# gitvicky/CP-PRE

Hardware: AMD Instinct MI355X
Metric: residual-cells/s (PRE eval+calibrate) (higher is better)
Workload: dtype f32

## Files before the change

cp_pre_amd/csrc/star_march.h:

```cpp
#pragma once
#include "common.h"
#include "host_checks.h"
#include <atomic>
#include <type_traits>

namespace {

constexpr int MAXF = 6;

struct Geom {
    const float *f[MAXF];
    long long sB[MAXF], sT[MAXF], sX[MAXF];
    float *out;
    long long oB, oT, oX;
    int B, T, X, Y;
    int Yc;
    int tSeg, nTSeg, nXT, nYT;
    int flags;
    int flat;
    int tfree;
    int obuf;
};

struct Star { float c, tm, tp, xm, xp, ym, yp; };

struct Nbr { float4 c, tm, tp, xm, xp, ym, yp; };

__device__ __forceinline__ float4 f4(float s) { return make_float4(s, s, s, s); }
__device__ __forceinline__ float4 fabs4(const float4 &a) { return make_float4(fabsf(a.x), fabsf(a.y), fabsf(a.z), fabsf(a.w)); }

enum Kind { K_T3, K_X3, K_Y3, K_XY5, K_TX5, K_STAR7, K_TY5 };

template <int KIND>
__device__ __forceinline__ float4 apply(const Star &w, const Nbr &n)
{
    if (KIND == K_T3) return w.tm * n.tm + w.c * n.c + w.tp * n.tp;
    if (KIND == K_X3) return w.xm * n.xm + w.c * n.c + w.xp * n.xp;
    if (KIND == K_Y3) return w.ym * n.ym + w.c * n.c + w.yp * n.yp;
    if (KIND == K_XY5) return w.xm * n.xm + w.ym * n.ym + w.c * n.c + w.yp * n.yp + w.xp * n.xp;
    if (KIND == K_TX5) return w.tm * n.tm + w.xm * n.xm + w.c * n.c + w.xp * n.xp + w.tp * n.tp;
    if (KIND == K_TY5) return w.tm * n.tm + w.ym * n.ym + w.c * n.c + w.yp * n.yp + w.tp * n.tp;
    const float4 tm = w.tm != 0.f ? w.tm * n.tm : f4(0.f), tp = w.tp != 0.f ? w.tp * n.tp : f4(0.f);
    return tm + w.xm * n.xm + w.ym * n.ym + w.c * n.c + w.yp * n.yp + w.xp * n.xp + tp;
}

template <int MODE> struct OpKinds {
    static constexpr int DT = MODE == 2 ? K_STAR7 : (MODE >= 3 ? K_Y3 : K_T3);
    static constexpr int DX = MODE == 2 ? K_STAR7 : (MODE >= 3 ? K_T3 : K_X3);
    static constexpr int DY = MODE == 2 ? K_STAR7 : (MODE == 0 ? K_T3 : MODE == 1 ? K_Y3 : MODE == 3 ? K_Y3 : K_X3);
    static constexpr int LAP = MODE == 2 ? K_STAR7 : (MODE >= 3 ? K_TX5 : K_XY5);
};

enum { O_DT = 1, O_DX = 2, O_DY = 4, O_LAP = 8 };
constexpr bool kind_has_x(int k) { return k == K_X3 || k == K_XY5 || k == K_TX5 || k == K_STAR7; }
template <int MODE> constexpr bool ops_have_x(int ops)
{
    using K = OpKinds<MODE>;
    return ((ops & O_DT) && kind_has_x(K::DT)) || ((ops & O_DX) && kind_has_x(K::DX)) || ((ops & O_DY) && kind_has_x(K::DY)) ||
           ((ops & O_LAP) && kind_has_x(K::LAP));
}
template <int MODE> constexpr unsigned xmask_of(int o0, int o1 = 0, int o2 = 0, int o3 = 0, int o4 = 0, int o5 = 0)
{
    return (ops_have_x<MODE>(o0) ? 1u : 0u) | (ops_have_x<MODE>(o1) ? 2u : 0u) | (ops_have_x<MODE>(o2) ? 4u : 0u) |
           (ops_have_x<MODE>(o3) ? 8u : 0u) | (ops_have_x<MODE>(o4) ? 16u : 0u) | (ops_have_x<MODE>(o5) ? 32u : 0u);
}

struct Linear1 {
    static constexpr int F = 1;
    struct Params { Star s; };
    static __device__ __forceinline__ float4 eval(const Nbr (&n)[1], const Params &p) { return apply<K_STAR7>(p.s, n[0]); }
};

struct Linear2 {
    static constexpr int F = 2;
    struct Params { Star a, b; float ratio; };
    static __device__ __forceinline__ float4 eval(const Nbr (&n)[2], const Params &p)
    {
        return apply<K_STAR7>(p.a, n[0]) + p.ratio * apply<K_STAR7>(p.b, n[1]);
    }
};

struct NSParams { Star Dt, Dx, Dy, L; float dxdy, dtdy, dtdx, nudt; };
struct BurgersParams { Star Dt, Dx, Dxx; float dx, dt, nu, c3; };
struct MHDParams { Star Dt, Dx, Dy; float gamma, gm2; };

template <int MODE>
struct NSMomentum {
    static constexpr int F = 3;
    static constexpr int MIN_WAVES = MODE >= 3 ? 4 : 1;
    static constexpr bool HALO_LEAD = MODE == 0;
    static constexpr unsigned XMASK = xmask_of<MODE>(O_DT | O_DX | O_DY | O_LAP, O_DT | O_DX | O_DY | O_LAP, O_DX | O_DY);
    using Params = NSParams;
    static __device__ __forceinline__ float4 eval(const Nbr (&n)[3], const Params &p)
    {
        using K = OpKinds<MODE>;
        const Nbr &u = n[0], &v = n[1], &pr = n[2];
        float4 rx = apply<K::DT>(p.Dt, u) * p.dxdy;
        rx = rx + u.c * apply<K::DX>(p.Dx, u) * p.dtdy;
        rx = rx + v.c * apply<K::DY>(p.Dy, u) * p.dtdx;
        rx = rx - apply<K::LAP>(p.L, u) * p.nudt;
        rx = rx + apply<K::DX>(p.Dx, pr) * p.dtdy;
        float4 ry = apply<K::DT>(p.Dt, v) * p.dxdy;
        ry = ry + u.c * apply<K::DX>(p.Dx, v) * p.dtdx;
        ry = ry + v.c * apply<K::DY>(p.Dy, v) * p.dtdy;
        ry = ry - apply<K::LAP>(p.L, v) * p.nudt;
        ry = ry + apply<K::DY>(p.Dy, pr) * p.dtdx;
        return rx + ry;
    }
};

template <int MODE>
struct Burgers {
    static constexpr int F = 1;
    using Params = BurgersParams;
    static __device__ __forceinline__ float4 eval(const Nbr (&n)[1], const Params &p)
    {
        constexpr int KT = MODE == 0 ? K_X3 : MODE == 3 ? K_Y3 : K_STAR7, KX = MODE == 0 ? K_Y3 : MODE == 3 ? K_X3 : K_STAR7;
        const Nbr &u = n[0];
        float4 r = p.dx * apply<KT>(p.Dt, u);
        r = r + (p.dt * u.c) * apply<KX>(p.Dx, u);
        r = r - (p.nu * apply<KX>(p.Dxx, u)) * p.c3;
        return r;
    }
};

template <int MODE>
struct MHDContinuity {
    static constexpr int F = 3;
    static constexpr unsigned XMASK = xmask_of<MODE>(O_DT | O_DX | O_DY, O_DX, O_DY);
    using Params = MHDParams;
    static __device__ __forceinline__ float4 eval(const Nbr (&n)[3], const Params &p)
    {
        using K = OpKinds<MODE>;
        const Nbr &rho = n[0], &u = n[1], &v = n[2];
        float4 r = apply<K::DT>(p.Dt, rho) + u.c * apply<K::DX>(p.Dx, rho);
        r = r + rho.c * apply<K::DX>(p.Dx, u);
        r = r + v.c * apply<K::DY>(p.Dy, rho);
        r = r + rho.c * apply<K::DY>(p.Dy, v);
        return r;
    }
};

template <int MODE>
struct MHDMomentum {
    static constexpr int F = 6;
    static constexpr unsigned XMASK = xmask_of<MODE>(0, O_DT | O_DX | O_DY, O_DT | O_DX | O_DY, O_DX | O_DY, O_DX | O_DY, O_DX | O_DY);
    using Params = MHDParams;
    static __device__ __forceinline__ float4 eval(const Nbr (&n)[6], const Params &p)
    {
        using K = OpKinds<MODE>;
        const Nbr &rho = n[0], &u = n[1], &v = n[2], &pr = n[3], &bx = n[4], &by = n[5];
        const float4 irho = f4(1.0f) / rho.c, bxr = bx.c / rho.c, byr = by.c / rho.c;
        float4 rx = apply<K::DT>(p.Dt, u) + u.c * apply<K::DX>(p.Dx, u);
        rx = rx + irho * apply<K::DX>(p.Dx, pr);
        rx = rx - (2.0f * bxr) * apply<K::DX>(p.Dx, bx);
        rx = rx + v.c * apply<K::DY>(p.Dy, u);
        rx = rx - byr * apply<K::DY>(p.Dy, bx);
        rx = rx - bxr * apply<K::DY>(p.Dy, by);
        float4 ry = apply<K::DT>(p.Dt, v) + u.c * apply<K::DX>(p.Dx, v);
        ry = ry + irho * apply<K::DY>(p.Dy, pr);
        ry = ry - (2.0f * byr) * apply<K::DY>(p.Dy, by);
        ry = ry + v.c * apply<K::DY>(p.Dy, v);
        ry = ry - byr * apply<K::DX>(p.Dx, bx);
        ry = ry - bxr * apply<K::DX>(p.Dx, by);
        return rx + ry;
    }
};

template <int MODE>
struct MHDEnergy {
    static constexpr int F = 6;
    static constexpr unsigned XMASK = xmask_of<MODE>(O_DT, O_DX | O_DY, O_DX | O_DY, O_DX | O_DY, O_DX, O_DY);
    using Params = MHDParams;
    static __device__ __forceinline__ float4 eval(const Nbr (&n)[6], const Params &p)
    {
        using K = OpKinds<MODE>;
        const Nbr &rho = n[0], &u = n[1], &v = n[2], &pr = n[3], &bx = n[4], &by = n[5];
        const float4 bx2 = bx.c * bx.c, by2 = by.c * by.c;
        const float4 pgas = pr.c - 0.5f * (bx2 + by2);
        float4 r = apply<K::DT>(p.Dt, rho) + u.c * apply<K::DX>(p.Dx, pr);
        r = r + v.c * apply<K::DY>(p.Dy, pr);
        r = r + (p.gm2 * (u.c * bx.c + v.c * by.c)) * (apply<K::DX>(p.Dx, bx) + apply<K::DY>(p.Dy, by));
        r = r + (p.gamma * pgas + by2) * apply<K::DX>(p.Dx, u);
        r = r + (p.gamma * pgas + bx2) * apply<K::DY>(p.Dy, v);
        r = r - (bx.c * by.c) * (apply<K::DY>(p.Dy, u) + apply<K::DX>(p.Dx, v));
        return r;
    }
};

template <int MODE>
struct MHDInduction {
    static constexpr int F = 4;
    static constexpr unsigned XMASK = xmask_of<MODE>(O_DX | O_DY, O_DX | O_DY, O_DT | O_DX | O_DY, O_DT | O_DX | O_DY);
    using Params = MHDParams;
    static __device__ __forceinline__ float4 eval(const Nbr (&n)[4], const Params &p)
    {
        using K = OpKinds<MODE>;
        const Nbr &u = n[0], &v = n[1], &bx = n[2], &by = n[3];
        float4 rx = apply<K::DT>(p.Dt, bx) - by.c * apply<K::DY>(p.Dy, u);
        rx = rx + bx.c * apply<K::DY>(p.Dy, v);
        rx = rx - v.c * apply<K::DY>(p.Dy, bx);
        rx = rx + u.c * apply<K::DY>(p.Dy, by);
        float4 ry = apply<K::DT>(p.Dt, by) + by.c * apply<K::DX>(p.Dx, u);
        ry = ry - bx.c * apply<K::DX>(p.Dx, v);
        ry = ry - v.c * apply<K::DX>(p.Dx, bx);
        ry = ry + u.c * apply<K::DX>(p.Dx, by);
        return rx + ry;
    }
};

struct JorekParams { Star Dt, DR, DZ, DRR, DZZ; float a0, a1, a2, a3; };

template <int MODE>
struct JorekContinuity {
    static constexpr int F = 3;
    static constexpr unsigned XMASK = xmask_of<MODE>(O_DT | O_DX | O_DY, O_DX | O_DY, 0);
    using Params = JorekParams;
    static __device__ __forceinline__ float4 eval(const Nbr (&n)[3], const Params &p)
    {
        using K = OpKinds<MODE>;
        const Nbr &rho = n[0], &phi = n[1];
        const float4 R = n[2].c;
        const float4 dRrho = apply<K::DX>(p.DR, rho), dZphi = apply<K::DY>(p.DZ, phi);
        const float4 X = dRrho * dZphi - apply<K::DX>(p.DR, phi) * apply<K::DY>(p.DZ, rho);
        const float4 Y = (apply<K::DX>(p.DRR, rho) + (f4(1.0f) / R) * dRrho) + apply<K::DY>(p.DZZ, rho);
        float4 r = p.a0 * apply<K::DT>(p.Dt, rho);
        r = r - (p.a1 * R) * X;
        r = r - (p.a2 * rho.c) * dZphi;
        r = r - p.a3 * Y;
        return r;
    }
};

template <int MODE>
struct JorekTemperature {
    static constexpr int F = 4;
    static constexpr unsigned XMASK = xmask_of<MODE>(O_DT | O_DX | O_DY, O_DX | O_DY, O_DT | O_DX | O_DY, 0);
    using Params = JorekParams;
    static __device__ __forceinline__ float4 eval(const Nbr (&n)[4], const Params &p)
    {
        using K = OpKinds<MODE>;
        const Nbr &rho = n[0], &phi = n[1], &T = n[2];
        const float4 R = n[3].c;
        const float4 dZphi = apply<K::DY>(p.DZ, phi), dRphi = apply<K::DX>(p.DR, phi);
        const float4 dRT = apply<K::DX>(p.DR, T);
        const float4 XT = dRT * dZphi - dRphi * apply<K::DY>(p.DZ, T);
        const float4 Xr = apply<K::DX>(p.DR, rho) * dZphi - dRphi * apply<K::DY>(p.DZ, rho);
        const float4 YT = (apply<K::DX>(p.DRR, T) + (f4(1.0f) / R) * dRT) + apply<K::DY>(p.DZZ, T);
        float4 r = T.c * apply<K::DT>(p.Dt, rho) + rho.c * apply<K::DT>(p.Dt, T);
        r = r - (rho.c * R) * XT;
        r = r + (T.c * R) * Xr;
        r = r + ((p.a0 * rho.c) * T.c) * dZphi;
        r = r + p.a3 * YT;
        return r;
    }
};

struct __attribute__((aligned(4))) F4u { float x, y, z, w; };
__device__ __forceinline__ float4 ldg4(const float *p)
{
    const F4u v = *reinterpret_cast<const F4u *>(p);
    return make_float4(v.x, v.y, v.z, v.w);
}
__device__ __forceinline__ void stg4(float *p, const float4 &r) { *reinterpret_cast<F4u *>(p) = F4u{r.x, r.y, r.z, r.w}; }

#ifndef MARCH_ST_SC1
#define MARCH_ST_SC1 0
#endif
__device__ __forceinline__ void stb4_sc1(float *plane, unsigned int off, const float4 &r)
{
    typedef unsigned int u32x4 __attribute__((ext_vector_type(4)));
    const u32x4 v = {__float_as_uint(r.x), __float_as_uint(r.y), __float_as_uint(r.z), __float_as_uint(r.w)};
    __builtin_amdgcn_raw_buffer_store_b128(v, __builtin_amdgcn_make_buffer_rsrc(plane, 0, -1, 0x00020000), (int)off, 0, 16);
}

#ifndef MARCH_DPP
#define MARCH_DPP 0
#endif
__device__ __forceinline__ float lane_below(float x)
{
#if MARCH_DPP
    return __int_as_float(__builtin_amdgcn_update_dpp(0, __float_as_int(x), 0x138, 0xf, 0xf, false));
#else
    return __shfl_up(x, 1);
#endif
}
__device__ __forceinline__ float lane_above(float x)
{
#if MARCH_DPP
    return __int_as_float(__builtin_amdgcn_update_dpp(0, __float_as_int(x), 0x130, 0xf, 0xf, false));
#else
    return __shfl_down(x, 1);
#endif
}

__device__ __forceinline__ void lds_barrier()
{
    __builtin_amdgcn_fence(__ATOMIC_RELEASE, "workgroup", "local");
    __builtin_amdgcn_s_barrier();
    __builtin_amdgcn_fence(__ATOMIC_ACQUIRE, "workgroup", "local");
}

template <int F, bool BC, bool COOP> struct Halo {
    typename std::conditional<COOP, float, float4>::type row[F];
    float ye[F];
    float yr[BC ? F : 1];
};

struct NoBC {};

#ifndef MARCH6_NR
#define MARCH6_NR 8
#endif
#ifndef MARCH6_TYQ
#define MARCH6_TYQ 64
#endif
#ifndef MARCH6_MINW
#define MARCH6_MINW 1
#endif
#ifndef MARCH1_TSEG
#define MARCH1_TSEG 0
#endif
#ifndef MARCHN_TSEG
#define MARCHN_TSEG 0
#endif
#ifndef TFREE_TSEG
#define TFREE_TSEG 8
#endif
#ifndef MARCH1_ANYB
#define MARCH1_ANYB 0
#endif
#ifndef MARCH6_AHEAD
#define MARCH6_AHEAD 2
#endif
#ifndef MARCH_COOP_MAXF
#define MARCH_COOP_MAXF 4
#endif
#ifndef MARCH_HALO_AHEAD
#define MARCH_HALO_AHEAD 1
#endif
#ifndef MARCH_NS16
#define MARCH_NS16 0
#endif

template <class Fn, class = void> struct MinWaves { static constexpr int value = Fn::F >= 5 ? MARCH6_MINW : 1; };
template <class Fn> struct MinWaves<Fn, std::void_t<decltype(Fn::MIN_WAVES)>> { static constexpr int value = Fn::MIN_WAVES; };

template <class Fn, class = void> struct HaloLead { static constexpr bool value = MARCH_HALO_AHEAD == 2; };
template <class Fn> struct HaloLead<Fn, std::void_t<decltype(Fn::HALO_LEAD)>> {
    static constexpr bool value = MARCH_HALO_AHEAD == 2 || (MARCH_HALO_AHEAD == 1 && Fn::HALO_LEAD);
};

template <class Fn, class = void> struct XMask { static constexpr unsigned value = (1u << Fn::F) - 1u; };
template <class Fn> struct XMask<Fn, std::void_t<decltype(Fn::XMASK)>> { static constexpr unsigned value = Fn::XMASK & ((1u << Fn::F) - 1u); };
template <class Fn> struct Staged {
    static constexpr unsigned M = XMask<Fn>::value;
    static constexpr int count = __builtin_popcount(M);
    static constexpr int FX = count > 0 ? count : 1;
    static __device__ __forceinline__ constexpr bool has(int i) { return (M >> i) & 1u; }
    static __device__ __forceinline__ constexpr int slot(int i) { return __builtin_popcount(M & ((1u << i) - 1u)); }
};

template <class Fn, int NR, int TYQ, bool BC = false>
__global__ void __launch_bounds__(NR *TYQ, MinWaves<Fn>::value)
march_kernel(const Geom g, const typename Fn::Params prm, const typename std::conditional<BC, BCInfo, NoBC>::type bc)
{
    constexpr int F = Fn::F;
    using SX = Staged<Fn>;
    constexpr int AHEAD = (F >= 5 && MARCH6_AHEAD == 3) ? 3 : 2;
    constexpr bool HAL3 = HaloLead<Fn>::value && !BC && F <= MARCH_COOP_MAXF && AHEAD == 2;
    static_assert(NR >= 2, "tile needs at least two rows (top and bottom halo owners differ)");
    __shared__ float4 lds[2][SX::FX][NR + 2][TYQ];

    const int q = threadIdx.x, ty = threadIdx.y;
    unsigned L = xcd_remap(blockIdx.x, gridDim.x);
    const int yt = L % g.nYT; L /= g.nYT;
    const int xt = L % g.nXT; L /= g.nXT;
    const int ts = L % g.nTSeg;
    const int b = L / g.nTSeg;

    const int x = xt * NR + ty, y = (yt * TYQ + q) * 4;
    const bool inb = (x < g.X) && (y < g.Yc);
    int xl = x;
    float ghost = 0.f;
    bool ldown = inb;
    if constexpr (BC) {
        if (x == g.X && y < g.Yc) { xl = bc.xhi; ghost = bc.vxhi; ldown = bc.xhi >= 0; }
    } else {
        if ((g.flags & PRE_FLAG_HALO_X) && x == g.X && y < g.Yc) ldown = true;
    }
    int t0 = ts * g.tSeg;
    int t1 = min(t0 + g.tSeg, g.T);
    if (g.flags & PRE_FLAG_INTERIOR_T) {
        t0 = max(t0, 1);
        t1 = min(t1, g.T - 1);
    }

    static_assert(NR >= 8 && (4 * TYQ) % 64 == 0, "the two halo rows are fetched by the first 8*TYQ threads, a wave per 64 floats");
    constexpr bool COOP = F <= MARCH_COOP_MAXF;
    const int hl = ty * TYQ + q;
    const bool hduty = COOP ? hl < 8 * TYQ : (ty == 0 || ty == NR - 1), hbot = COOP ? hl >= 4 * TYQ : ty == NR - 1;
    const int hcol = COOP ? hl & (4 * TYQ - 1) : 4 * q;
    const int hy = yt * (4 * TYQ) + hcol;
    int hx = hbot ? xt * NR + NR : xt * NR - 1;
    const bool halox = (g.flags & PRE_FLAG_HALO_X) != 0;
    bool hrow = hduty && (halox ? (hx >= -1 && hx <= g.X) : (hx >= 0 && hx < g.X)) && (hy < g.Yc);
    float hfill = 0.f;
    const int hslot = hbot ? NR + 1 : 0;
    const bool ledge = ((q & 63) == 0);
    bool redge = ((q & 63) == 63) || (q == TYQ - 1);
    bool lload = ledge && inb && (y > 0);
    bool rload = redge && inb && (y + 4 < g.Y);
    int yloff = -1, yroff = 4;
    float ylfill = 0.f, yrfill = 0.f;
    const bool tailq = !BC && (x < g.X) && (y >= g.Yc) && (y < g.Y);
    if constexpr (BC) {
        if (hduty && hy < g.Yc && (hx == -1 || hx == g.X)) {
            const int m = hx < 0 ? bc.xlo : bc.xhi;
            hfill = hx < 0 ? bc.vxlo : bc.vxhi;
            hrow = m >= 0;
            hx = m >= 0 ? m : 0;
        }
        if (inb && y == 0) { lload = bc.ylo >= 0; yloff = bc.ylo; ylfill = bc.vylo; }
        if (inb && y + 4 >= g.Y) { redge = true; rload = bc.yhi >= 0; yroff = bc.yhi - y; yrfill = bc.vyhi; }
    }
    const bool eload = BC ? lload : (ledge ? lload : rload);
    const int eoff4 = 4 * (BC ? yloff : (ledge ? yloff : yroff));
    const float efill = BC ? ylfill : 0.f;

    unsigned int voff[F], hoff[F];
#pragma unroll
    for (int i = 0; i < F; ++i) {
        voff[i] = (unsigned int)(((long long)(xl + 1) * g.sX[i] + y) * 4);
        hoff[i] = (unsigned int)(((long long)(hx + 1) * g.sX[i] + hy) * 4);
    }
    constexpr bool SC1 = MARCH_ST_SC1 != 0;
    const long long oel = (long long)x * g.oX + y;
    const unsigned int ooff = (unsigned int)(oel * 4);
    float *outp = g.out + (long long)b * g.oB + (SC1 ? 0 : oel);
    const long long oT = g.oT;
    const int tlo = g.tfree ? t0 : 0, thi = g.tfree ? t1 : g.T;
    typedef unsigned int u32x4 __attribute__((ext_vector_type(4)));
    auto plane = [&](int i, int t) __attribute__((always_inline)) {
        const float *p = g.f[i] + ((long long)b * g.sB[i] - g.sX[i] + (long long)t * g.sT[i]);
        return __builtin_amdgcn_make_buffer_rsrc(const_cast<float *>(p), 0, -1, 0x00020000);
    };

    auto load_own = [&](int t, float4(&dst)[F]) __attribute__((always_inline)) {
        const bool ok = ldown && (t >= tlo) && (t < thi);
#pragma unroll
        for (int i = 0; i < F; ++i) {
            if (ok) {
                const u32x4 v = __builtin_amdgcn_raw_buffer_load_b128(plane(i, t), (int)voff[i], 0, 0);
                dst[i] = make_float4(__uint_as_float(v.x), __uint_as_float(v.y), __uint_as_float(v.z), __uint_as_float(v.w));
            } else {
                dst[i] = f4(BC ? ghost : 0.f);
                if (tailq && (t >= tlo) && (t < thi))
                    dst[i].x = __uint_as_float(__builtin_amdgcn_raw_buffer_load_b32(plane(i, t), (int)voff[i], 0, 0));
            }
        }
    };
    auto load_halo = [&](int t, Halo<F, BC, COOP> &h) __attribute__((always_inline)) {
        const bool okt = (t >= tlo) && (t < thi);
#pragma unroll
        for (int i = 0; i < F; ++i) {
            if (!SX::has(i)) {
                if constexpr (COOP) h.row[i] = 0.f; else h.row[i] = f4(0.f);
            } else if constexpr (COOP) {
                h.row[i] = (hrow && okt) ? __uint_as_float(__builtin_amdgcn_raw_buffer_load_b32(plane(i, t), (int)hoff[i], 0, 0))
                                         : (BC ? hfill : 0.f);
            } else if (hrow && okt) {
                const u32x4 v = __builtin_amdgcn_raw_buffer_load_b128(plane(i, t), (int)hoff[i], 0, 0);
                h.row[i] = make_float4(__uint_as_float(v.x), __uint_as_float(v.y), __uint_as_float(v.z), __uint_as_float(v.w));
            } else {
                h.row[i] = f4(BC ? hfill : 0.f);
            }
            h.ye[i] = (eload && okt) ? __uint_as_float(__builtin_amdgcn_raw_buffer_load_b32(plane(i, t), (int)voff[i] + eoff4, 0, 0))
                                     : (BC ? efill : 0.f);
            if constexpr (BC)
                h.yr[i] = (rload && okt) ? __uint_as_float(__builtin_amdgcn_raw_buffer_load_b32(plane(i, t), (int)voff[i] + 4 * yroff, 0, 0))
                                         : yrfill;
        }
    };

    auto step = [&](int t, float4(&P)[F], float4(&C)[F], float4(&N)[F], float4(&D)[F],
                    Halo<F, BC, COOP> &hc, Halo<F, BC, COOP> &hn) __attribute__((always_inline)) {
        const int bi = (t - t0) & 1;
#pragma unroll
        for (int i = 0; i < F; ++i) {
            if (!SX::has(i)) continue;
            const int k = SX::slot(i);
            lds[bi][k][ty + 1][q] = C[i];
            if constexpr (COOP) {
                if (hduty) reinterpret_cast<float *>(&lds[bi][k][hslot][0])[hcol] = hc.row[i];
            } else {
                if (hduty) lds[bi][k][hslot][q] = hc.row[i];
            }
        }
        load_halo(t + (HAL3 ? AHEAD : 1), hn);
        load_own(t + AHEAD, D);
        if constexpr (SX::count > 0) lds_barrier();

        Nbr n[F];
#pragma unroll
        for (int i = 0; i < F; ++i) {
            n[i].c = C[i];
            n[i].tm = P[i];
            n[i].tp = N[i];
            if (SX::has(i)) {
                n[i].xm = lds[bi][SX::slot(i)][ty][q];
                n[i].xp = lds[bi][SX::slot(i)][ty + 2][q];
            } else {
                n[i].xm = n[i].xp = f4(__builtin_nanf(""));
            }
            float lft = lane_below(C[i].w);
            float rgt = lane_above(C[i].x);
            lft = ledge ? hc.ye[i] : lft;
            rgt = redge ? (BC ? hc.yr[i] : hc.ye[i]) : rgt;
            n[i].ym = make_float4(lft, C[i].x, C[i].y, C[i].z);
            n[i].yp = make_float4(C[i].y, C[i].z, C[i].w, rgt);
        }
        float4 r = Fn::eval(n, prm);
        if (g.flags & PRE_FLAG_ABS) r = fabs4(r);
        if (inb) {
            if constexpr (SC1) {
                if (g.obuf) stb4_sc1(outp + (long long)t * oT, ooff, r);
                else stg4(outp + (long long)t * oT + ((long long)x * g.oX + y), r);
            } else {
                stg4(outp + (long long)t * oT, r);
            }
        }
    };

    Halo<F, BC, COOP> h0, h1;
    if constexpr (AHEAD == 3) {
        float4 w0[F], w1[F], w2[F], w3[F], w4[F];
        load_own(t0 - 1, w0);
        load_own(t0, w1);
        load_own(t0 + 1, w2);
        load_own(t0 + 2, w3);
        load_halo(t0, h0);
        for (int t = t0; t < t1; t += 5) {
            step(t, w0, w1, w2, w4, h0, h1);
            if (t + 1 >= t1) break;
            step(t + 1, w1, w2, w3, w0, h1, h0);
            if (t + 2 >= t1) break;
            step(t + 2, w2, w3, w4, w1, h0, h1);
            if (t + 3 >= t1) break;
            step(t + 3, w3, w4, w0, w2, h1, h0);
            if (t + 4 >= t1) break;
            step(t + 4, w4, w0, w1, w3, h0, h1);
            h0 = h1;
        }
    } else if constexpr (HAL3) {
        float4 w0[F], w1[F], w2[F], w3[F];
        Halo<F, BC, COOP> h2;
        load_own(t0 - 1, w0);
        load_own(t0, w1);
        load_own(t0 + 1, w2);
        load_halo(t0, h0);
        load_halo(t0 + 1, h1);
        for (int t = t0; t < t1; t += 12) {
            step(t, w0, w1, w2, w3, h0, h2);
            if (t + 1 >= t1) break;
            step(t + 1, w1, w2, w3, w0, h1, h0);
            if (t + 2 >= t1) break;
            step(t + 2, w2, w3, w0, w1, h2, h1);
            if (t + 3 >= t1) break;
            step(t + 3, w3, w0, w1, w2, h0, h2);
            if (t + 4 >= t1) break;
            step(t + 4, w0, w1, w2, w3, h1, h0);
            if (t + 5 >= t1) break;
            step(t + 5, w1, w2, w3, w0, h2, h1);
            if (t + 6 >= t1) break;
            step(t + 6, w2, w3, w0, w1, h0, h2);
            if (t + 7 >= t1) break;
            step(t + 7, w3, w0, w1, w2, h1, h0);
            if (t + 8 >= t1) break;
            step(t + 8, w0, w1, w2, w3, h2, h1);
            if (t + 9 >= t1) break;
            step(t + 9, w1, w2, w3, w0, h0, h2);
            if (t + 10 >= t1) break;
            step(t + 10, w2, w3, w0, w1, h1, h0);
            if (t + 11 >= t1) break;
            step(t + 11, w3, w0, w1, w2, h2, h1);
        }
    } else {
        float4 w0[F], w1[F], w2[F], w3[F];
        load_own(t0 - 1, w0);
        load_own(t0, w1);
        load_own(t0 + 1, w2);
        load_halo(t0, h0);
        for (int t = t0; t < t1; t += 4) {
            step(t, w0, w1, w2, w3, h0, h1);
            if (t + 1 >= t1) break;
            step(t + 1, w1, w2, w3, w0, h1, h0);
            if (t + 2 >= t1) break;
            step(t + 2, w2, w3, w0, w1, h0, h1);
            if (t + 3 >= t1) break;
            step(t + 3, w3, w0, w1, w2, h1, h0);
        }
    }
}

bool star_from_dense27(const float *K, Star *s)
{
    auto at = [&](int a, int b, int c) { return K[(a * 3 + b) * 3 + c]; };
    for (int a = 0; a < 3; ++a)
        for (int b = 0; b < 3; ++b)
            for (int c = 0; c < 3; ++c) {
                const int off = (a != 1) + (b != 1) + (c != 1);
                if (off > 1 && at(a, b, c) != 0.0f) return false;
            }
    s->c = at(1, 1, 1);
    s->tm = at(0, 1, 1); s->tp = at(2, 1, 1);
    s->xm = at(1, 0, 1); s->xp = at(1, 2, 1);
    s->ym = at(1, 1, 0); s->yp = at(1, 1, 2);
    return true;
}

bool star_of_taps(const float *w, const int32_t *off, int ntaps, Star *s, int *rc)
{
    float s7[7] = {0, 0, 0, 0, 0, 0, 0};
    bool star = true;
    *rc = PRE_OK;
    for (int i = 0; i < ntaps; ++i) {
        const int dt = off[3 * i], dx = off[3 * i + 1], dy = off[3 * i + 2];
        if (dt < -3 || dt > 3 || dx < -3 || dx > 3 || dy < -3 || dy > 3) { *rc = PRE_E_SHAPE; return false; }
        const int nz = (dt != 0) + (dx != 0) + (dy != 0);
        if (nz > 1 || dt < -1 || dt > 1 || dx < -1 || dx > 1 || dy < -1 || dy > 1) { star = false; continue; }
        const int slot = dt ? (dt < 0 ? 1 : 2) : dx ? (dx < 0 ? 3 : 4) : dy ? (dy < 0 ? 5 : 6) : 0;
        s7[slot] += w[i];
    }
    *s = Star{s7[0], s7[1], s7[2], s7[3], s7[4], s7[5], s7[6]};
    return star;
}

struct Shape { bool t, x, y; };
Shape shape_of(const Star &s) { return {s.tm != 0.f || s.tp != 0.f, s.xm != 0.f || s.xp != 0.f, s.ym != 0.f || s.yp != 0.f}; }

int pick_mode(const Star &Dt, const Star &Dx, const Star &Dy, const Star *L)
{
    const Shape st = shape_of(Dt), sx = shape_of(Dx), sy = shape_of(Dy);
    const bool dt_ok = !st.x && !st.y, dx_ok = !sx.t && !sx.y;
    const bool lap_ok = !L || !shape_of(*L).t;
    if (dt_ok && dx_ok && lap_ok && !sy.x && !sy.y) return 0;
    if (dt_ok && dx_ok && lap_ok && !sy.x && !sy.t) return 1;
    return 2;
}

int chip_cus()
{
    static const int cus = [] {
        int dev = 0, n = 0;
        if (hipGetDevice(&dev) != hipSuccess || hipDeviceGetAttribute(&n, hipDeviceAttributeMultiprocessorCount, dev) != hipSuccess || n <= 0) n = 256;
        return n;
    }();
    return cus;
}

template <class K> int resident_per_cu(K kernel, int threads)
{
    int n = 0;
    if (hipOccupancyMaxActiveBlocksPerMultiprocessor(&n, kernel, threads, 0) != hipSuccess || n < 1) n = 1;
    return n;
}

int pick_tseg(long long tiles, int T, long long slots)
{
    int best = T;
    double bestc = 1e300;
    for (int tSeg = T;; tSeg = (tSeg + 1) / 2) {
        const long long wgs = tiles * ((T + tSeg - 1) / tSeg);
        const double rounds = (double)wgs / (double)slots;
        const double full = (rounds <= 1.0 ? 1.0 : (double)((wgs + slots - 1) / slots)) + 0.5;
        const double cost = (1.0 + 3.0 / tSeg) * full / rounds;
        if (cost < bestc * 0.99) { best = tSeg; bestc = cost; }
        if (tSeg <= 16) break;
    }
    return best;
}

template <class Fn, int NR, int TYQ, bool BC = false>
int launch_tiled(Geom &g, const typename Fn::Params &prm, hipStream_t st, const BCInfo *bc = nullptr)
{
    static_assert(2 * Staged<Fn>::FX * (NR + 2) * TYQ * 16 <= 160 * 1024, "tile does not fit the 160 KiB LDS");
    {
    g.nXT = (g.X + NR - 1) / NR;
    g.nYT = (g.Yc + 4 * TYQ - 1) / (4 * TYQ);
    for (int i = 0; i < Fn::F; ++i)
        if (!plane_offsets_fit_u32(g.sX[i], (int64_t)g.X + 2 + NR, g.Y)) return PRE_E_UNSUPPORTED;
    g.obuf = MARCH_ST_SC1 != 0 && plane_offsets_fit_u32(g.oX, (int64_t)g.X + NR, g.Y);
    long long tiles = (long long)g.B * g.nXT * g.nYT;
    static const int per_cu = resident_per_cu(march_kernel<Fn, NR, TYQ, BC>, NR * TYQ);
    int tSeg = pick_tseg(tiles, g.T, (long long)per_cu * chip_cus());
    if (MARCH1_TSEG > 0 && Fn::F == 1 && (g.B > 1 || MARCH1_ANYB) && g.T >= 4 * MARCH1_TSEG && tSeg > MARCH1_TSEG) tSeg = MARCH1_TSEG;
    if (TFREE_TSEG > 0 && g.tfree && tSeg > TFREE_TSEG) tSeg = TFREE_TSEG;
    if (MARCHN_TSEG > 0 && tSeg > MARCHN_TSEG) tSeg = MARCHN_TSEG;
    g.tSeg = tSeg;
    g.nTSeg = (g.T + tSeg - 1) / tSeg;
    tiles *= g.nTSeg;
    if (tiles <= 0 || tiles * TYQ > 0xffffffffLL) return PRE_E_SHAPE;
    if constexpr (BC) {
        hipLaunchKernelGGL((march_kernel<Fn, NR, TYQ, true>), dim3((unsigned)tiles), dim3(TYQ, NR), 0, st, g, prm, *bc);
    } else {
        hipLaunchKernelGGL((march_kernel<Fn, NR, TYQ, false>), dim3((unsigned)tiles), dim3(TYQ, NR), 0, st, g, prm, NoBC{});
    }
    PRE_LAUNCH_CHECK();
    return PRE_OK;
    }
}

#ifndef FLAT_MAX_Y
#define FLAT_MAX_Y 96
#endif
#ifndef FLAT_Q4
#define FLAT_Q4 0
#endif
#ifndef FLAT_SYNC
#define FLAT_SYNC 0
#endif

#ifndef FLAT_STAGE_ALL
#define FLAT_STAGE_ALL 0
#endif
template <class Fn> struct AllStaged {
    static constexpr int count = Fn::F, FX = Fn::F;
    static __device__ __forceinline__ constexpr bool has(int) { return true; }
    static __device__ __forceinline__ constexpr int slot(int i) { return i; }
};
template <class Fn> using FlatStaged = typename std::conditional<FLAT_STAGE_ALL != 0, AllStaged<Fn>, Staged<Fn>>::type;

template <int F> struct FlatHalo {
    float4 q[F];
    float e[F];
};

template <class Fn, bool Q4>
__global__ void __launch_bounds__(FLAT_NT, MinWaves<Fn>::value)
flat_march_kernel(const Geom g, const typename Fn::Params prm)
{
    constexpr int F = Fn::F;
    using SX = FlatStaged<Fn>;
    constexpr bool ANY = SX::count > 0;
    __shared__ float4 lds[2][SX::FX][ANY ? FLAT_NT + 2 * FLAT_H : 1];
    const int q = threadIdx.x;
    unsigned Lb = xcd_remap(blockIdx.x, gridDim.x);
    const int ch = Lb % g.nYT; Lb /= g.nYT;
    const int ts = Lb % g.nTSeg;
    const int b = Lb / g.nTSeg;
    const int Ty = g.Y, L = g.X * g.Y;
    const int NT = blockDim.x;
    const int m0 = ch * NT * 4, m = m0 + 4 * q;
    const bool inb = m < L;
    int t0 = ts * g.tSeg, t1 = min(t0 + g.tSeg, g.T);
    if (g.flags & PRE_FLAG_INTERIOR_T) {
        t0 = max(t0, 1);
        t1 = min(t1, g.T - 1);
    }

    const int HQ = FLAT_HALO_FULL ? FLAT_H : min(FLAT_H, (Ty + 3) >> 2);
    const bool hl = q < HQ, hr = q >= NT - HQ;
    const int hm = hl ? m0 - 4 * (HQ - q) : m0 + 4 * NT + 4 * (q - (NT - HQ));
    const bool hok = (hl || hr) && hm >= 0 && hm < L;
    const int hslot = hl ? FLAT_H - HQ + q : FLAT_H + NT + (q - (NT - HQ));

    bool lok[4], rok[4];
    {
        int ph = m % Ty;
#pragma unroll
        for (int j = 0; j < 4; ++j) {
            lok[j] = (Q4 && j > 0) || ph != 0;
            rok[j] = (Q4 && j < 3) || ph != Ty - 1;
            ph = ph + 1 == Ty ? 0 : ph + 1;
        }
    }
    const bool ledge = (q & 63) == 0, redge = (q & 63) == 63;
    const bool eload = inb && (ledge ? lok[0] : (redge && rok[3]));

    const unsigned int voff = (unsigned int)m * 4u, hoff = (unsigned int)hm * 4u;
    const unsigned int eoff = ledge ? voff - 4u : voff + 16u;
    constexpr bool SC1 = MARCH_ST_SC1 != 0;
    float *outp = g.out + (long long)b * g.oB + (SC1 ? 0 : m);
    const long long oT = g.oT;
    typedef unsigned int u32x4 __attribute__((ext_vector_type(4)));
    auto rsrc = [&](int i, int t) __attribute__((always_inline)) {
        const float *p = g.f[i] + ((long long)b * g.sB[i] + (long long)t * g.sT[i]);
        return __builtin_amdgcn_make_buffer_rsrc(const_cast<float *>(p), 0, -1, 0x00020000);
    };
    auto quad = [&](int i, int t, unsigned int off) __attribute__((always_inline)) {
        const u32x4 v = __builtin_amdgcn_raw_buffer_load_b128(rsrc(i, t), (int)off, 0, 0);
        return make_float4(__uint_as_float(v.x), __uint_as_float(v.y), __uint_as_float(v.z), __uint_as_float(v.w));
    };

    auto load_own = [&](int t, float4(&dst)[F]) __attribute__((always_inline)) {
        const bool ok = inb && (t >= 0) && (t < g.T);
#pragma unroll
        for (int i = 0; i < F; ++i) {
            if (ok) dst[i] = quad(i, t, voff);
            else dst[i] = f4(0.f);
        }
    };
    auto load_halo = [&](int t, FlatHalo<F> &h) __attribute__((always_inline)) {
        const bool okt = (t >= 0) && (t < g.T);
#pragma unroll
        for (int i = 0; i < F; ++i) {
            if (SX::has(i)) {
                h.e[i] = 0.f;
                if (hok && okt) h.q[i] = quad(i, t, hoff);
                else h.q[i] = f4(0.f);
            } else {
                h.q[i] = f4(0.f);
                h.e[i] = (eload && okt) ? __uint_as_float(__builtin_amdgcn_raw_buffer_load_b32(rsrc(i, t), (int)eoff, 0, 0)) : 0.f;
            }
        }
    };

    auto step = [&](int t, float4(&P)[F], float4(&C)[F], float4(&N)[F], float4(&D)[F], FlatHalo<F> &hc,
                    FlatHalo<F> &hn) __attribute__((always_inline)) {
        const int bi = (t - t0) & 1;
#pragma unroll
        for (int i = 0; i < F; ++i) {
            if (!SX::has(i)) continue;
            const int k = SX::slot(i);
            lds[bi][k][FLAT_H + q] = C[i];
            if (hl || hr) lds[bi][k][hslot] = hc.q[i];
        }
        load_halo(t + 1, hn);
        load_own(t + 2, D);
        if constexpr (ANY) lds_barrier();
        else if (FLAT_SYNC) __builtin_amdgcn_s_barrier();

        Nbr n[F];
#pragma unroll
        for (int i = 0; i < F; ++i) {
            n[i].c = C[i];
            n[i].tm = P[i];
            n[i].tp = N[i];
            float lft, rgt;
            if (SX::has(i)) {
                const int k = SX::slot(i);
                const float *row = reinterpret_cast<const float *>(&lds[bi][k][0]) + 4 * (FLAT_H + q);
                if (Q4) {
                    n[i].xm = lds[bi][k][FLAT_H + q - (Ty >> 2)];
                    n[i].xp = lds[bi][k][FLAT_H + q + (Ty >> 2)];
                } else if ((Ty & 1) == 0) {
                    const float2 a = *reinterpret_cast<const float2 *>(row - Ty), b = *reinterpret_cast<const float2 *>(row + 2 - Ty);
                    const float2 c = *reinterpret_cast<const float2 *>(row + Ty), d = *reinterpret_cast<const float2 *>(row + 2 + Ty);
                    n[i].xm = make_float4(a.x, a.y, b.x, b.y);
                    n[i].xp = make_float4(c.x, c.y, d.x, d.y);
                } else {
// ... 172 lines not shown
```

Before: 299.5 billion.

## Add boustrophedon time-segment marching with grouped tile ordering for seam reuse

Odd time segments now march backward, so adjacent segments start at a shared seam plane that the neighbouring workgroup has just read and that may still sit in L2. Tiles are regrouped so that the segments of one spatial window are scheduled close together. Fields with no time taps no longer load the extra seam planes. A new cost model picks the segment length and group size (Linear1 defaults to 4 segments), replacing the old fixed TSEG overrides. The price is more complex index decoding, selects for the march direction, and possible changes to occupancy or register use.

```diff
diff --git a/cp_pre_amd/csrc/star_march.h b/cp_pre_amd/csrc/star_march.h
--- a/cp_pre_amd/csrc/star_march.h
+++ b/cp_pre_amd/csrc/star_march.h
@@ -19,6 +19,8 @@
     int flags;
     int flat;
     int tfree;
+    int seam;
+    int gT;
     int obuf;
 };
 
@@ -27,6 +29,7 @@
 struct Nbr { float4 c, tm, tp, xm, xp, ym, yp; };
 
 __device__ __forceinline__ float4 f4(float s) { return make_float4(s, s, s, s); }
+__device__ __forceinline__ float4 sel4(bool c, float4 a, float4 b) { return make_float4(c ? a.x : b.x, c ? a.y : b.y, c ? a.z : b.z, c ? a.w : b.w); }
 __device__ __forceinline__ float4 fabs4(const float4 &a) { return make_float4(fabsf(a.x), fabsf(a.y), fabsf(a.z), fabsf(a.w)); }
 
 enum Kind { K_T3, K_X3, K_Y3, K_XY5, K_TX5, K_STAR7, K_TY5 };
@@ -65,8 +68,29 @@
            (ops_have_x<MODE>(o3) ? 8u : 0u) | (ops_have_x<MODE>(o4) ? 16u : 0u) | (ops_have_x<MODE>(o5) ? 32u : 0u);
 }
 
+constexpr bool kind_has_t(int k) { return k == K_T3 || k == K_TX5 || k == K_TY5 || k == K_STAR7; }
+template <int MODE> constexpr bool ops_have_t(int ops)
+{
+    using K = OpKinds<MODE>;
+    return ((ops & O_DT) && kind_has_t(K::DT)) || ((ops & O_DX) && kind_has_t(K::DX)) || ((ops & O_DY) && kind_has_t(K::DY)) ||
+           ((ops & O_LAP) && kind_has_t(K::LAP));
+}
+template <int MODE> constexpr unsigned tmask_of(int o0, int o1 = 0, int o2 = 0, int o3 = 0, int o4 = 0, int o5 = 0)
+{
+    return (ops_have_t<MODE>(o0) ? 1u : 0u) | (ops_have_t<MODE>(o1) ? 2u : 0u) | (ops_have_t<MODE>(o2) ? 4u : 0u) |
+           (ops_have_t<MODE>(o3) ? 8u : 0u) | (ops_have_t<MODE>(o4) ? 16u : 0u) | (ops_have_t<MODE>(o5) ? 32u : 0u);
+}
+
+#ifndef MARCH_NS_SEAM_SEGS
+#define MARCH_NS_SEAM_SEGS -1
+#endif
+#ifndef MARCH_L1_SEAM_SEGS
+#define MARCH_L1_SEAM_SEGS 4
+#endif
+
 struct Linear1 {
     static constexpr int F = 1;
+    static constexpr int SEAM_SEGS = MARCH_L1_SEAM_SEGS;
     struct Params { Star s; };
     static __device__ __forceinline__ float4 eval(const Nbr (&n)[1], const Params &p) { return apply<K_STAR7>(p.s, n[0]); }
 };
@@ -89,7 +113,9 @@
     static constexpr int F = 3;
     static constexpr int MIN_WAVES = MODE >= 3 ? 4 : 1;
     static constexpr bool HALO_LEAD = MODE == 0;
+    static constexpr int SEAM_SEGS = MODE == 0 ? MARCH_NS_SEAM_SEGS : -1;
     static constexpr unsigned XMASK = xmask_of<MODE>(O_DT | O_DX | O_DY | O_LAP, O_DT | O_DX | O_DY | O_LAP, O_DX | O_DY);
+    static constexpr unsigned TMASK = tmask_of<MODE>(O_DT | O_DX | O_DY | O_LAP, O_DT | O_DX | O_DY | O_LAP, O_DX | O_DY);
     using Params = NSParams;
     static __device__ __forceinline__ float4 eval(const Nbr (&n)[3], const Params &p)
     {
@@ -128,6 +154,7 @@
 struct MHDContinuity {
     static constexpr int F = 3;
     static constexpr unsigned XMASK = xmask_of<MODE>(O_DT | O_DX | O_DY, O_DX, O_DY);
+    static constexpr unsigned TMASK = tmask_of<MODE>(O_DT | O_DX | O_DY, O_DX, O_DY);
     using Params = MHDParams;
     static __device__ __forceinline__ float4 eval(const Nbr (&n)[3], const Params &p)
     {
@@ -145,6 +172,7 @@
 struct MHDMomentum {
     static constexpr int F = 6;
     static constexpr unsigned XMASK = xmask_of<MODE>(0, O_DT | O_DX | O_DY, O_DT | O_DX | O_DY, O_DX | O_DY, O_DX | O_DY, O_DX | O_DY);
+    static constexpr unsigned TMASK = tmask_of<MODE>(0, O_DT | O_DX | O_DY, O_DT | O_DX | O_DY, O_DX | O_DY, O_DX | O_DY, O_DX | O_DY);
     using Params = MHDParams;
     static __device__ __forceinline__ float4 eval(const Nbr (&n)[6], const Params &p)
     {
@@ -171,6 +199,7 @@
 struct MHDEnergy {
     static constexpr int F = 6;
     static constexpr unsigned XMASK = xmask_of<MODE>(O_DT, O_DX | O_DY, O_DX | O_DY, O_DX | O_DY, O_DX, O_DY);
+    static constexpr unsigned TMASK = tmask_of<MODE>(O_DT, O_DX | O_DY, O_DX | O_DY, O_DX | O_DY, O_DX, O_DY);
     using Params = MHDParams;
     static __device__ __forceinline__ float4 eval(const Nbr (&n)[6], const Params &p)
     {
@@ -192,6 +221,7 @@
 struct MHDInduction {
     static constexpr int F = 4;
     static constexpr unsigned XMASK = xmask_of<MODE>(O_DX | O_DY, O_DX | O_DY, O_DT | O_DX | O_DY, O_DT | O_DX | O_DY);
+    static constexpr unsigned TMASK = tmask_of<MODE>(O_DX | O_DY, O_DX | O_DY, O_DT | O_DX | O_DY, O_DT | O_DX | O_DY);
     using Params = MHDParams;
     static __device__ __forceinline__ float4 eval(const Nbr (&n)[4], const Params &p)
     {
@@ -215,6 +245,7 @@
 struct JorekContinuity {
     static constexpr int F = 3;
     static constexpr unsigned XMASK = xmask_of<MODE>(O_DT | O_DX | O_DY, O_DX | O_DY, 0);
+    static constexpr unsigned TMASK = tmask_of<MODE>(O_DT | O_DX | O_DY, O_DX | O_DY, 0);
     using Params = JorekParams;
     static __device__ __forceinline__ float4 eval(const Nbr (&n)[3], const Params &p)
     {
@@ -236,6 +267,7 @@
 struct JorekTemperature {
     static constexpr int F = 4;
     static constexpr unsigned XMASK = xmask_of<MODE>(O_DT | O_DX | O_DY, O_DX | O_DY, O_DT | O_DX | O_DY, 0);
+    static constexpr unsigned TMASK = tmask_of<MODE>(O_DT | O_DX | O_DY, O_DX | O_DY, O_DT | O_DX | O_DY, 0);
     using Params = JorekParams;
     static __device__ __forceinline__ float4 eval(const Nbr (&n)[4], const Params &p)
     {
@@ -318,17 +350,8 @@
 #ifndef MARCH6_MINW
 #define MARCH6_MINW 1
 #endif
-#ifndef MARCH1_TSEG
-#define MARCH1_TSEG 0
-#endif
-#ifndef MARCHN_TSEG
-#define MARCHN_TSEG 0
-#endif
 #ifndef TFREE_TSEG
 #define TFREE_TSEG 8
-#endif
-#ifndef MARCH1_ANYB
-#define MARCH1_ANYB 0
 #endif
 #ifndef MARCH6_AHEAD
 #define MARCH6_AHEAD 2
@@ -361,6 +384,16 @@
     static __device__ __forceinline__ constexpr int slot(int i) { return __builtin_popcount(M & ((1u << i) - 1u)); }
 };
 
+template <class Fn, class = void> struct TMask { static constexpr unsigned value = (1u << Fn::F) - 1u; };
+template <class Fn> struct TMask<Fn, std::void_t<decltype(Fn::TMASK)>> { static constexpr unsigned value = Fn::TMASK & ((1u << Fn::F) - 1u); };
+template <class Fn> struct TTapped {
+    static __device__ __host__ __forceinline__ constexpr bool has(int i) { return (TMask<Fn>::value >> i) & 1u; }
+    static constexpr int count = __builtin_popcount(TMask<Fn>::value);
+};
+
+template <class Fn, class = void> struct SeamSegs { static constexpr bool can = false; static constexpr int value = 0; };
+template <class Fn> struct SeamSegs<Fn, std::void_t<decltype(Fn::SEAM_SEGS)>> { static constexpr bool can = Fn::SEAM_SEGS >= 0; static constexpr int value = Fn::SEAM_SEGS; };
+
 template <class Fn, int NR, int TYQ, bool BC = false>
 __global__ void __launch_bounds__(NR *TYQ, MinWaves<Fn>::value)
 march_kernel(const Geom g, const typename Fn::Params prm, const typename std::conditional<BC, BCInfo, NoBC>::type bc)
@@ -373,11 +406,14 @@
     __shared__ float4 lds[2][SX::FX][NR + 2][TYQ];
 
     const int q = threadIdx.x, ty = threadIdx.y;
-    unsigned L = xcd_remap(blockIdx.x, gridDim.x);
-    const int yt = L % g.nYT; L /= g.nYT;
-    const int xt = L % g.nXT; L /= g.nXT;
-    const int ts = L % g.nTSeg;
-    const int b = L / g.nTSeg;
+    const unsigned L = xcd_remap(blockIdx.x, gridDim.x);
+    const unsigned tpp = (unsigned)(g.nXT * g.nYT), per = tpp * (unsigned)g.nTSeg;
+    const int b = L / per;
+    const unsigned r = L - (unsigned)b * per;
+    const unsigned gbase = r / ((unsigned)g.gT * g.nTSeg) * g.gT, gsz = min((unsigned)g.gT, tpp - gbase), rr = r - gbase * g.nTSeg;
+    const int ts = rr / gsz;
+    const unsigned tile = gbase + (rr - (unsigned)ts * gsz);
+    const int yt = tile % g.nYT, xt = tile / g.nYT;
 
     const int x = xt * NR + ty, y = (yt * TYQ + q) * 4;
     const bool inb = (x < g.X) && (y < g.Yc);
@@ -439,7 +475,12 @@
     const unsigned int ooff = (unsigned int)(oel * 4);
     float *outp = g.out + (long long)b * g.oB + (SC1 ? 0 : oel);
     const long long oT = g.oT;
-    const int tlo = g.tfree ? t0 : 0, thi = g.tfree ? t1 : g.T;
+    using TT = TTapped<Fn>;
+    const int tlo0 = t0, thi0 = t1;
+    const int tlo1 = g.tfree ? t0 : max(t0 - 1, 0), thi1 = g.tfree ? t1 : min(t1 + 1, g.T);
+    constexpr bool SEAMS = SeamSegs<Fn>::can && !BC;
+    const bool down = SEAMS && g.seam && (ts & 1);
+    const int dir = down ? -1 : 1, ts0 = down ? t1 - 1 : t0, nst = t1 - t0;
     typedef unsigned int u32x4 __attribute__((ext_vector_type(4)));
     auto plane = [&](int i, int t) __attribute__((always_inline)) {
         const float *p = g.f[i] + ((long long)b * g.sB[i] - g.sX[i] + (long long)t * g.sT[i]);
@@ -447,23 +488,25 @@
     };
 
     auto load_own = [&](int t, float4(&dst)[F]) __attribute__((always_inline)) {
-        const bool ok = ldown && (t >= tlo) && (t < thi);
+        const bool in0 = (t >= tlo0) && (t < thi0), in1 = (t >= tlo1) && (t < thi1);
 #pragma unroll
         for (int i = 0; i < F; ++i) {
-            if (ok) {
+            const bool okt = TT::has(i) ? in1 : in0;
+            if (ldown && okt) {
                 const u32x4 v = __builtin_amdgcn_raw_buffer_load_b128(plane(i, t), (int)voff[i], 0, 0);
                 dst[i] = make_float4(__uint_as_float(v.x), __uint_as_float(v.y), __uint_as_float(v.z), __uint_as_float(v.w));
             } else {
                 dst[i] = f4(BC ? ghost : 0.f);
-                if (tailq && (t >= tlo) && (t < thi))
+                if (tailq && okt)
                     dst[i].x = __uint_as_float(__builtin_amdgcn_raw_buffer_load_b32(plane(i, t), (int)voff[i], 0, 0));
             }
         }
     };
     auto load_halo = [&](int t, Halo<F, BC, COOP> &h) __attribute__((always_inline)) {
-        const bool okt = (t >= tlo) && (t < thi);
+        const bool in0 = (t >= tlo0) && (t < thi0), in1 = (t >= tlo1) && (t < thi1);
 #pragma unroll
         for (int i = 0; i < F; ++i) {
+            const bool okt = TT::has(i) ? in1 : in0;
             if (!SX::has(i)) {
                 if constexpr (COOP) h.row[i] = 0.f; else h.row[i] = f4(0.f);
             } else if constexpr (COOP) {
@@ -483,30 +526,37 @@
         }
     };
 
-    auto step = [&](int t, float4(&P)[F], float4(&C)[F], float4(&N)[F], float4(&D)[F],
+    auto step = [&](int k, float4(&P)[F], float4(&C)[F], float4(&N)[F], float4(&D)[F],
                     Halo<F, BC, COOP> &hc, Halo<F, BC, COOP> &hn) __attribute__((always_inline)) {
-        const int bi = (t - t0) & 1;
+        const int bi = k & 1, t = ts0 + k * dir;
 #pragma unroll
         for (int i = 0; i < F; ++i) {
             if (!SX::has(i)) continue;
-            const int k = SX::slot(i);
-            lds[bi][k][ty + 1][q] = C[i];
+            const int sl = SX::slot(i);
+            lds[bi][sl][ty + 1][q] = C[i];
             if constexpr (COOP) {
-                if (hduty) reinterpret_cast<float *>(&lds[bi][k][hslot][0])[hcol] = hc.row[i];
+                if (hduty) reinterpret_cast<float *>(&lds[bi][sl][hslot][0])[hcol] = hc.row[i];
             } else {
-                if (hduty) lds[bi][k][hslot][q] = hc.row[i];
+                if (hduty) lds[bi][sl][hslot][q] = hc.row[i];
             }
         }
-        load_halo(t + (HAL3 ? AHEAD : 1), hn);
-        load_own(t + AHEAD, D);
+        load_halo(t + (HAL3 ? AHEAD : 1) * dir, hn);
+        load_own(t + AHEAD * dir, D);
         if constexpr (SX::count > 0) lds_barrier();
 
         Nbr n[F];
 #pragma unroll
         for (int i = 0; i < F; ++i) {
             n[i].c = C[i];
-            n[i].tm = P[i];
-            n[i].tp = N[i];
+            if (!TT::has(i)) {
+                n[i].tm = n[i].tp = f4(__builtin_nanf(""));
+            } else if constexpr (SEAMS) {
+                n[i].tm = sel4(down, N[i], P[i]);
+                n[i].tp = sel4(down, P[i], N[i]);
+            } else {
+                n[i].tm = P[i];
+                n[i].tp = N[i];
+            }
             if (SX::has(i)) {
                 n[i].xm = lds[bi][SX::slot(i)][ty][q];
                 n[i].xp = lds[bi][SX::slot(i)][ty + 2][q];
@@ -535,70 +585,70 @@
     Halo<F, BC, COOP> h0, h1;
     if constexpr (AHEAD == 3) {
         float4 w0[F], w1[F], w2[F], w3[F], w4[F];
-        load_own(t0 - 1, w0);
-        load_own(t0, w1);
-        load_own(t0 + 1, w2);
-        load_own(t0 + 2, w3);
-        load_halo(t0, h0);
-        for (int t = t0; t < t1; t += 5) {
-            step(t, w0, w1, w2, w4, h0, h1);
-            if (t + 1 >= t1) break;
-            step(t + 1, w1, w2, w3, w0, h1, h0);
-            if (t + 2 >= t1) break;
-            step(t + 2, w2, w3, w4, w1, h0, h1);
-            if (t + 3 >= t1) break;
-            step(t + 3, w3, w4, w0, w2, h1, h0);
-            if (t + 4 >= t1) break;
-            step(t + 4, w4, w0, w1, w3, h0, h1);
+        load_own(ts0 - dir, w0);
+        load_own(ts0, w1);
+        load_own(ts0 + dir, w2);
+        load_own(ts0 + 2 * dir, w3);
+        load_halo(ts0, h0);
+        for (int k = 0; k < nst; k += 5) {
+            step(k, w0, w1, w2, w4, h0, h1);
+            if (k + 1 >= nst) break;
+            step(k + 1, w1, w2, w3, w0, h1, h0);
+            if (k + 2 >= nst) break;
+            step(k + 2, w2, w3, w4, w1, h0, h1);
+            if (k + 3 >= nst) break;
+            step(k + 3, w3, w4, w0, w2, h1, h0);
+            if (k + 4 >= nst) break;
+            step(k + 4, w4, w0, w1, w3, h0, h1);
             h0 = h1;
         }
     } else if constexpr (HAL3) {
         float4 w0[F], w1[F], w2[F], w3[F];
         Halo<F, BC, COOP> h2;
-        load_own(t0 - 1, w0);
-        load_own(t0, w1);
-        load_own(t0 + 1, w2);
-        load_halo(t0, h0);
-        load_halo(t0 + 1, h1);
-        for (int t = t0; t < t1; t += 12) {
-            step(t, w0, w1, w2, w3, h0, h2);
-            if (t + 1 >= t1) break;
-            step(t + 1, w1, w2, w3, w0, h1, h0);
-            if (t + 2 >= t1) break;
-            step(t + 2, w2, w3, w0, w1, h2, h1);
-            if (t + 3 >= t1) break;
-            step(t + 3, w3, w0, w1, w2, h0, h2);
-            if (t + 4 >= t1) break;
-            step(t + 4, w0, w1, w2, w3, h1, h0);
-            if (t + 5 >= t1) break;
-            step(t + 5, w1, w2, w3, w0, h2, h1);
-            if (t + 6 >= t1) break;
-            step(t + 6, w2, w3, w0, w1, h0, h2);
-            if (t + 7 >= t1) break;
-            step(t + 7, w3, w0, w1, w2, h1, h0);
-            if (t + 8 >= t1) break;
-            step(t + 8, w0, w1, w2, w3, h2, h1);
-            if (t + 9 >= t1) break;
-            step(t + 9, w1, w2, w3, w0, h0, h2);
-            if (t + 10 >= t1) break;
-            step(t + 10, w2, w3, w0, w1, h1, h0);
-            if (t + 11 >= t1) break;
-            step(t + 11, w3, w0, w1, w2, h2, h1);
+        load_own(ts0 - dir, w0);
+        load_own(ts0, w1);
+        load_own(ts0 + dir, w2);
+        load_halo(ts0, h0);
+        load_halo(ts0 + dir, h1);
+        for (int k = 0; k < nst; k += 12) {
+            step(k, w0, w1, w2, w3, h0, h2);
+            if (k + 1 >= nst) break;
+            step(k + 1, w1, w2, w3, w0, h1, h0);
+            if (k + 2 >= nst) break;
+            step(k + 2, w2, w3, w0, w1, h2, h1);
+            if (k + 3 >= nst) break;
+            step(k + 3, w3, w0, w1, w2, h0, h2);
+            if (k + 4 >= nst) break;
+            step(k + 4, w0, w1, w2, w3, h1, h0);
+            if (k + 5 >= nst) break;
+            step(k + 5, w1, w2, w3, w0, h2, h1);
+            if (k + 6 >= nst) break;
+            step(k + 6, w2, w3, w0, w1, h0, h2);
+            if (k + 7 >= nst) break;
+            step(k + 7, w3, w0, w1, w2, h1, h0);
+            if (k + 8 >= nst) break;
+            step(k + 8, w0, w1, w2, w3, h2, h1);
+            if (k + 9 >= nst) break;
+            step(k + 9, w1, w2, w3, w0, h0, h2);
+            if (k + 10 >= nst) break;
+            step(k + 10, w2, w3, w0, w1, h1, h0);
+            if (k + 11 >= nst) break;
+            step(k + 11, w3, w0, w1, w2, h2, h1);
         }
     } else {
         float4 w0[F], w1[F], w2[F], w3[F];
-        load_own(t0 - 1, w0);
-        load_own(t0, w1);
-        load_own(t0 + 1, w2);
-        load_halo(t0, h0);
-        for (int t = t0; t < t1; t += 4) {
-            step(t, w0, w1, w2, w3, h0, h1);
-            if (t + 1 >= t1) break;
-            step(t + 1, w1, w2, w3, w0, h1, h0);
-            if (t + 2 >= t1) break;
-            step(t + 2, w2, w3, w0, w1, h0, h1);
-            if (t + 3 >= t1) break;
-            step(t + 3, w3, w0, w1, w2, h1, h0);
+        load_own(ts0 - dir, w0);
+        load_own(ts0, w1);
+        load_own(ts0 + dir, w2);
+        load_halo(ts0, h0);
+        for (int k = 0; k < nst; k += 4) {
+            step(k, w0, w1, w2, w3, h0, h1);
+            if (k + 1 >= nst) break;
+            step(k + 1, w1, w2, w3, w0, h1, h0);
+            if (k + 2 >= nst) break;
+            step(k + 2, w2, w3, w0, w1, h0, h1);
+            if (k + 3 >= nst) break;
+            step(k + 3, w3, w0, w1, w2, h1, h0);
         }
     }
 }
@@ -681,6 +731,55 @@
     return best;
 }
 
+struct SeamPlan { int tSeg, nSeg, gT, seamsIn, seamsOut; };
+
+#ifndef MARCH_SEAM_GROUP
+#define MARCH_SEAM_GROUP 1
+#endif
+SeamPlan seam_plan(int T, int tSeg, int nXT, int nYT, long long win)
+{
+    SeamPlan p;
+    p.tSeg = tSeg;
+    p.nSeg = (T + tSeg - 1) / tSeg;
+    const long long tpp = (long long)nXT * nYT;
+    p.gT = (int)tpp;
+    if (MARCH_SEAM_GROUP && p.nSeg > 2 && tpp * p.nSeg > win && win / p.nSeg >= 4LL * nYT)
+        p.gT = (int)(win / p.nSeg / nYT * nYT);
+    p.seamsIn = p.seamsOut = 0;
+    for (int s = 0; s + 1 < p.nSeg; ++s) {
+        const bool in = win > 0 && ((long long)s * p.gT) / win == ((long long)(s + 2) * p.gT - 1) / win;
+        (in ? p.seamsIn : p.seamsOut) += 1;
+    }
+    return p;
+}
+
+#ifndef SEAM_L2_COST
+#define SEAM_L2_COST 0.5
+#endif
+double seam_cost(const SeamPlan &p, long long tiles, int T, long long slots, int F, int ft)
+{
+    const long long wgs = tiles * p.nSeg;
+    const double rounds = (double)wgs / (double)slots;
+    const double full = (rounds <= 1.0 ? 1.0 : (double)((wgs + slots - 1) / slots)) + 0.5;
+    const double seam = 2.0 * ft / ((double)T * (F + 1));
+    return (1.0 + seam * (p.seamsOut + SEAM_L2_COST * p.seamsIn)) * full / rounds;
+}
+
+SeamPlan pick_seam_plan(long long tiles, int T, int nXT, int nYT, long long slots, int F, int ft, int fullSegs)
+{
+    const long long win = slots / 8;
+    if (fullSegs > 1 && tiles >= 2 * slots && T >= 8 * fullSegs) return seam_plan(T, (T + fullSegs - 1) / fullSegs, nXT, nYT, win);
+    SeamPlan best = seam_plan(T, T, nXT, nYT, win);
+    double bestc = 1e300;
+    for (int tSeg = T;; tSeg = (tSeg + 1) / 2) {
+        const SeamPlan p = seam_plan(T, tSeg, nXT, nYT, win);
+        const double c = seam_cost(p, tiles, T, slots, F, ft);
+        if (c < bestc * 0.99) { best = p; bestc = c; }
+        if (tSeg <= 16) break;
+    }
+    return best;
+}
+
 template <class Fn, int NR, int TYQ, bool BC = false>
 int launch_tiled(Geom &g, const typename Fn::Params &prm, hipStream_t st, const BCInfo *bc = nullptr)
 {
@@ -693,10 +792,22 @@
     g.obuf = MARCH_ST_SC1 != 0 && plane_offsets_fit_u32(g.oX, (int64_t)g.X + NR, g.Y);
     long long tiles = (long long)g.B * g.nXT * g.nYT;
     static const int per_cu = resident_per_cu(march_kernel<Fn, NR, TYQ, BC>, NR * TYQ);
+    g.seam = 0;
+    g.gT = g.nXT * g.nYT;
+    if constexpr (SeamSegs<Fn>::can && !BC) if (!g.tfree) {
+        const SeamPlan p = pick_seam_plan(tiles, g.T, g.nXT, g.nYT, (long long)per_cu * chip_cus(), Fn::F, TTapped<Fn>::count, SeamSegs<Fn>::value);
+        g.seam = 1;
+        g.gT = p.gT;
+        g.tSeg = p.tSeg;
+        g.nTSeg = p.nSeg;
+        tiles *= g.nTSeg;
+        if (tiles <= 0 || tiles * TYQ > 0xffffffffLL) return PRE_E_SHAPE;
+        hipLaunchKernelGGL((march_kernel<Fn, NR, TYQ, false>), dim3((unsigned)tiles), dim3(TYQ, NR), 0, st, g, prm, NoBC{});
+        PRE_LAUNCH_CHECK();
+        return PRE_OK;
+    }
     int tSeg = pick_tseg(tiles, g.T, (long long)per_cu * chip_cus());
-    if (MARCH1_TSEG > 0 && Fn::F == 1 && (g.B > 1 || MARCH1_ANYB) && g.T >= 4 * MARCH1_TSEG && tSeg > MARCH1_TSEG) tSeg = MARCH1_TSEG;
     if (TFREE_TSEG > 0 && g.tfree && tSeg > TFREE_TSEG) tSeg = TFREE_TSEG;
-    if (MARCHN_TSEG > 0 && tSeg > MARCHN_TSEG) tSeg = MARCHN_TSEG;
     g.tSeg = tSeg;
     g.nTSeg = (g.T + tSeg - 1) / tSeg;
     tiles *= g.nTSeg;
```

Result: no change. 298.2 billion (-0.4%).
